# clvrai/mopa-rl

Measured on AMD Instinct MI355X. Metric: valid-state collision checks/sec, higher is better.
Workload: dtype f64; 1 GPU; SawyerPushObstacle-v0 state validity (FK + collision), 4096 envs/GPU x 256 states/env per step, states 50% uniform joint-box samples + 50% near-init N(0,0.3); envs_per_gpu=4096, states_per_env=256, parallelism=env-shard x1

## Files before the change

include/mopa_hip.h:

```cpp
#ifndef MOPA_HIP_H
#define MOPA_HIP_H
#include <stdint.h>

#ifdef __cplusplus
extern "C" {
#endif

#define MOPA_OK 0
#define MOPA_ERR_INVALID_ARG 1
#define MOPA_ERR_UNSUPPORTED 2
#define MOPA_ERR_HIP 3
#define MOPA_ERR_LIMIT 4

#define MOPA_PLAN_OK 0
#define MOPA_PLAN_NO_EXACT (-4)
#define MOPA_PLAN_INVALID_GOAL (-5)

#define MOPA_FAR 1.0e10

enum { MOPA_GEOM_PLANE = 0, MOPA_GEOM_SPHERE = 2, MOPA_GEOM_CAPSULE = 3, MOPA_GEOM_CYLINDER = 5, MOPA_GEOM_BOX = 6, MOPA_GEOM_MESH = 7 };
enum { MOPA_JNT_FREE = 0, MOPA_JNT_BALL = 1, MOPA_JNT_SLIDE = 2, MOPA_JNT_HINGE = 3 };

typedef struct MopaModel {
    int32_t nq, nbody, njnt, ngeom, npair;
// ... 71 lines not shown
                         const double *attached_dev , int64_t E, int32_t max_path, void *stream);
int mopa_scene_num_active(const MopaScene *scene);
int mopa_scene_active_idx(const MopaScene *scene, int32_t *out );
int mopa_scene_num_pairs(const MopaScene *scene);
int mopa_scene_lds_bytes(const MopaScene *scene);
int mopa_scene_valid_kernel(const MopaScene *scene, int64_t N, char *out, int32_t cap );
int mopa_scene_motion_kernel(const MopaScene *scene, int64_t N, char *out, int32_t cap );
int mopa_scene_k1_baked(const MopaScene *scene);
int mopa_scene_k1_export(const MopaSceneDesc *desc, int64_t *sizes , double *dbl, int32_t *ints, int32_t *tab, void *hdr,
                         uint64_t *fingerprint);
int mopa_scene_hdr_offset(const char *field);
int mopa_scene_k1_export_glued(const MopaSceneDesc *desc, int32_t body_a, int32_t body_b, int64_t *sizes , double *dbl, int32_t *ints,
                               int32_t *tab, void *hdr, uint64_t *fingerprint);
int mopa_k1_baked_fk_host(int index, int64_t n, const double *q_active, const double *qpos_env, double *out);
int mopa_k1_baked_resident_host(int index, int64_t n, const double *q_active, const double *qpos_env, double *out, int32_t *n_res);

int mopa_is_valid_batch(MopaScene *scene, const double *q_active_dev , const double *qpos_env_dev ,
                        int64_t N, int64_t samples_per_env, uint8_t *valid_dev , double *min_dist_dev ,
                        void *stream);
int mopa_is_valid_batch_counted(MopaScene *scene, const double *q_active_dev , const double *qpos_env_dev ,
                                int64_t N, int64_t samples_per_env, uint8_t *valid_dev , double *min_dist_dev ,
                                const int64_t *n_dev, void *stream);

int mopa_check_motion_batch(MopaScene *scene, const double *qa_dev , const double *qb_dev ,
                            const double *qpos_env_dev , int64_t N, int64_t samples_per_env,
                            uint8_t *valid_dev , void *stream);

int mopa_plan_batch(MopaScene *scene, const double *start_dev , const double *goal_dev , int64_t E,
                    const MopaPlanParams *params, double *path_dev , int32_t *path_len_dev ,
                    int32_t *status_dev , int64_t *n_checks_dev , void *stream);
// ... 395 lines not shown
```

mopa_rl_amd/_lib.py:

```python
from __future__ import annotations

import ctypes as C
import os
from typing import Optional

import numpy as np

_HERE = os.path.dirname(os.path.abspath(__file__))
LIB_PATH = os.environ.get("MOPA_HIP_LIB", os.path.join(_HERE, "csrc", "libmopa_hip.so"))

MOPA_OK = 0
MOPA_FAR = 1.0e10
PLAN_OK, PLAN_NO_EXACT, PLAN_INVALID_GOAL = 0, -4, -5

_dp = C.POINTER(C.c_double)
_ip = C.POINTER(C.c_int32)

EXPORTED_SYMBOLS = [
    "mopa_last_error", "mopa_version", "mopa_device_count", "mopa_scene_create", "mopa_scene_destroy",
    "mopa_scene_create_glued", "mopa_scene_glue", "mopa_glue_attach_batch", "mopa_glue_rows_batch", "mopa_scene_k1_export_glued",
    "mopa_scene_num_active", "mopa_scene_active_idx", "mopa_scene_num_pairs", "mopa_scene_lds_bytes", "mopa_scene_valid_kernel",
    "mopa_scene_motion_kernel",
    "mopa_scene_k1_baked", "mopa_scene_k1_export", "mopa_scene_hdr_offset", "mopa_k1_baked_fk_host", "mopa_k1_baked_resident_host",
    "mopa_is_valid_batch", "mopa_is_valid_batch_counted", "mopa_check_motion_batch", "mopa_plan_batch", "mopa_simplify_paths_batch", "mopa_simplify_paths_max_path", "mopa_shortcut_paths_batch", "mopa_shortcut_paths_max_path", "mopa_smooth_paths_batch", "mopa_smooth_paths_max_path",
    "mopa_plan_star_batch", "mopa_plan_star", "mopa_plan_star_k", "mopa_star_params_size",
    "mopa_plan_race_batch", "mopa_plan_race", "mopa_race_params_size", "mopa_pullback_batch", "mopa_is_valid_state", "mopa_plan",
    "mopa_planner_status", "mopa_debug_fk", "mopa_debug_pair_dist", "mopa_contacts_batch", "mopa_contacts_state",
    "mopa_contact_frames_batch", "mopa_contact_frames_state", "mopa_geom_frames_batch", "mopa_geom_frames_host",
    "mopa_env_create", "mopa_env_destroy", "mopa_env_obs_dim", "mopa_env_action_dim", "mopa_env_step_batch", "mopa_env_exec_batch", "mopa_env_desired_batch",
    "mopa_env_attach_dynamics", "mopa_env_attach_contacts", "mopa_env_set_contact_stats", "mopa_rollout_stage", "mopa_rollout_pool_pick", "mopa_rollout_step_size", "mopa_reuse_batch", "mopa_replay_append", "mopa_replay_sample", "mopa_ct_desc_size", "mopa_env_contact_arena", "mopa_env_dyn_dofs", "mopa_env_dyn_qvel_width", "mopa_env_dyn_forward_batch", "mopa_env_dyn_substeps_batch", "mopa_env_step_dyn_batch",
    "mopa_pusher_dyn_desc_size", "mopa_env_attach_pusher_dynamics", "mopa_env_set_pusher_stats", "mopa_env_pusher_substeps_batch",
    "mopa_env_step_pusher_batch", "mopa_env_set_contact_force",
    "mopa_ik_create", "mopa_ik_destroy", "mopa_ik_solve_batch", "mopa_ik_site_pose_batch", "mopa_ik_targets_batch",
    "mopa_ik_targets_pos_batch", "mopa_ik_displacement_pos_batch",
    "mopa_paths_unwrap_batch", "mopa_paths_unwrap_seam_batch", "mopa_paths_walk_batch", "mopa_paths_assemble_batch", "mopa_interpolate_batch",
]


# ... 230 lines not shown
    L.mopa_ik_destroy.restype = None
    L.mopa_ik_solve_batch.argtypes = [vp, C.c_int64, vp, vp, vp, C.c_double, C.c_int32, C.c_double, C.c_double, C.c_double, C.c_double,
                                      vp, vp, vp, vp]
    L.mopa_ik_site_pose_batch.argtypes = [vp, C.c_int64, vp, vp, vp, vp]
    L.mopa_ik_targets_batch.argtypes = [vp, C.c_int64, vp, vp, vp, C.c_int64, C.c_double, C.POINTER(C.c_double), C.POINTER(C.c_double), vp, vp, vp]
    L.mopa_ik_targets_pos_batch.argtypes = [vp, C.c_int64, vp, vp, C.c_int64, C.c_int32, C.c_double, C.POINTER(C.c_double), C.POINTER(C.c_double), vp, vp]
    L.mopa_ik_displacement_pos_batch.argtypes = [vp, C.c_int64, vp, vp, C.c_int64, C.c_int32, C.c_double, C.POINTER(C.c_double), C.POINTER(C.c_double),
                                                 C.c_int32, C.c_double, C.c_double, C.c_double, C.c_double, vp, vp, vp, vp, vp, vp, vp]
    L.mopa_scene_valid_kernel.argtypes = [vp, C.c_int64, C.c_char_p, C.c_int32]
    L.mopa_scene_motion_kernel.argtypes = [vp, C.c_int64, C.c_char_p, C.c_int32]
    L.mopa_scene_k1_baked.argtypes = [vp]
    L.mopa_scene_k1_export.argtypes = [vp, vp, vp, vp, vp, vp, vp]
    L.mopa_scene_hdr_offset.argtypes = [C.c_char_p]
    L.mopa_k1_baked_fk_host.argtypes = [C.c_int, C.c_int64, vp, vp, vp]
    L.mopa_k1_baked_resident_host.argtypes = [C.c_int, C.c_int64, vp, vp, vp, vp]
    i32, i64, f64 = C.c_int32, C.c_int64, C.c_double
    L.mopa_paths_unwrap_batch.argtypes = [C.c_int, i64, i32, i32, vp, i32, vp, vp, vp, f64, i32, vp, vp, vp, vp, vp, vp, vp, vp]
    L.mopa_paths_unwrap_seam_batch.argtypes = [C.c_int, i64, i32, i32, vp, i32, vp, vp, vp, f64, i32, vp, vp, vp, vp, vp, vp, vp, C.c_uint64, vp]
    L.mopa_paths_walk_batch.argtypes = [C.c_int, i64, i32, i32, vp, i32, vp, vp, f64, vp, vp, vp, vp, vp, vp, vp, vp]
    L.mopa_paths_assemble_batch.argtypes = [C.c_int, i64, i32, vp, i32, vp, vp, vp, vp, vp, vp, vp, i32, vp, vp]
    L.mopa_interpolate_batch.argtypes = [vp, i64, i32, i32, vp, vp, f64, vp, vp, vp, vp, vp]
    _lib = L
    return L


def check(rc: int) -> None:
    if rc != MOPA_OK:
        raise MopaError(f"libmopa_hip error {rc}: {lib().mopa_last_error().decode()}")


# ... 344 lines not shown
```

mopa_rl_amd/csrc/mopa_hip.hip:

```cpp
#include <hip/hip_runtime.h>

#include <algorithm>
#include <cmath>
#include <cstdio>
#include <cstdlib>
#include <cstddef>
#include <cstring>
#include <string>
#include <utility>
#include <vector>

#include <map>
#include <mutex>
#include "../../include/mopa_hip.h"
#include "mopa_device.hpp"
#include "mopa_frames.hpp"
#include "mopa_fk.hpp"
#include "mopa_host.hpp"

using namespace mopa;

static thread_local std::string g_err;
int mopa_fail(int code, const std::string &msg) {
    g_err = msg;
// ... 482 lines not shown
extern "C" int mopa_scene_k1_export_glued(const MopaSceneDesc *desc, int32_t body_a, int32_t body_b, int64_t *sizes, double *dbl, int32_t *ints,
                                          int32_t *tab, void *hdr, uint64_t *fingerprint) {
    if (body_a < 0 || body_b < 0) return fail(MOPA_ERR_INVALID_ARG, "glue: body id out of range");
    return scene_k1_export(desc, body_a, body_b, sizes, dbl, ints, tab, hdr, fingerprint);
}

extern "C" int mopa_scene_hdr_offset(const char *field) {
    if (!field) return -1;
#define MOPA_HDR_FIELD(f_) if (!std::strcmp(field, #f_)) return (int)offsetof(SceneHdr, f_);
    MOPA_HDR_FIELD(na) MOPA_HDR_FIELD(nq) MOPA_HDR_FIELD(n_pq) MOPA_HDR_FIELD(nmb) MOPA_HDR_FIELD(nmg) MOPA_HDR_FIELD(nsf)
    MOPA_HDR_FIELD(n_save) MOPA_HDR_FIELD(n_pas_b) MOPA_HDR_FIELD(n_dbl) MOPA_HDR_FIELD(n_int) MOPA_HDR_FIELD(o_mbr) MOPA_HDR_FIELD(o_mbd)
    MOPA_HDR_FIELD(o_mgd) MOPA_HDR_FIELD(o_sf_pos) MOPA_HDR_FIELD(o_sf_quat) MOPA_HDR_FIELD(o_sf_mat) MOPA_HDR_FIELD(o_act_ref)
    MOPA_HDR_FIELD(o_pq_adr) MOPA_HDR_FIELD(o_mg_geom) MOPA_HDR_FIELD(thr)
    MOPA_HDR_FIELD(o_mb_parent) MOPA_HDR_FIELD(o_chain_adr) MOPA_HDR_FIELD(o_chain_len) MOPA_HDR_FIELD(o_chain_items) MOPA_HDR_FIELD(o_g_mb)
    MOPA_HDR_FIELD(o_mb_load) MOPA_HDR_FIELD(o_mb_save) MOPA_HDR_FIELD(pfk_maxlen) MOPA_HDR_FIELD(n_gp) MOPA_HDR_FIELD(npair) MOPA_HDR_FIELD(o_pairs)
    MOPA_HDR_FIELD(o_g_rec) MOPA_HDR_FIELD(o_g_type)
#undef MOPA_HDR_FIELD
    return -1;
}

namespace {
struct K1HostSink {
    double *out;
    void operator()(int m, V3 gp, Q4 gq) {
        double *o = out + 12 * m;
        o[0] = gp.x; o[1] = gp.y; o[2] = gp.z;
        quat2mat(o + 3, gq);
    }
    void resident(int, double) {}
};
struct K1ResHostSink {
    double *out;
    void operator()(int, V3, Q4) {}
    void resident(int r, double d) { out[r] = d; }
};
template <class TR>
void k1_fk_host(int64_t n, const double *q_active, const double *qpos_env, double *out) {
    for (int64_t s = 0; s < n; s++) {
        K1HostSink sink{out + (size_t)s * 12 * TR::nmg};
        k1_fk_baked<TR>(q_active + (size_t)s * TR::na, qpos_env + (size_t)s * TR::nq, sink, std::make_integer_sequence<int, TR::nmb>{});
    }
}
template <class TR>
void k1_res_host(int64_t n, const double *q_active, const double *qpos_env, double *out) {
    for (int64_t s = 0; s < n; s++) {
        K1ResHostSink sink{out + (size_t)s * k1_n_res<TR>};
        k1_fk_baked<TR>(q_active + (size_t)s * TR::na, qpos_env + (size_t)s * TR::nq, sink, std::make_integer_sequence<int, TR::nmb>{});
    }
}
}
extern "C" int mopa_k1_baked_fk_host(int index, int64_t n, const double *q_active, const double *qpos_env, double *out) {
    if (n < 0 || (n > 0 && (!q_active || !qpos_env || !out))) return fail(MOPA_ERR_INVALID_ARG, "null argument / negative count");
#define MOPA_K1_FK_HOST(i_, T_) if (index == i_) { k1_fk_host<T_>(n, q_active, qpos_env, out); return MOPA_OK; }
    MOPA_K1_BAKED_SCENES(MOPA_K1_FK_HOST)
#undef MOPA_K1_FK_HOST
    return fail(MOPA_ERR_INVALID_ARG, "no baked scene #" + std::to_string(index));
}
extern "C" int mopa_k1_baked_resident_host(int index, int64_t n, const double *q_active, const double *qpos_env, double *out, int32_t *n_res) {
    if (n < 0 || (n > 0 && (!q_active || !qpos_env || !out))) return fail(MOPA_ERR_INVALID_ARG, "null argument / negative count");
#define MOPA_K1_RES_HOST(i_, T_) if (index == i_) { if (n_res) *n_res = k1_n_res<T_>; if (k1_n_res<T_> > 0) k1_res_host<T_>(n, q_active, qpos_env, out); return MOPA_OK; }
    MOPA_K1_BAKED_SCENES(MOPA_K1_RES_HOST)
#undef MOPA_K1_RES_HOST
    return fail(MOPA_ERR_INVALID_ARG, "no baked scene #" + std::to_string(index));
}

static int scene_create(const MopaSceneDesc *desc, int glue_a, int glue_b, MopaScene **out) {
    if (!desc || !out) return fail(MOPA_ERR_INVALID_ARG, "null argument");
    MopaScene *S = new MopaScene();
    {
        const int rc = scene_build_host(desc, S, glue_a, glue_b);
        if (rc != MOPA_OK) { delete S; return rc; }
    }
    {
        const char *eb = std::getenv("MOPA_K1_BAKED");
        const uint64_t fp = k1_fingerprint(S);
        const bool allowed = !(eb && std::string(eb) == "0") && S->k1.use_v5 && S->k1.v5_cen_lds && S->n_mesh_gp == 0 && S->glue_b < 0;
        S->k1_baked = allowed ? k1_baked_index(fp) : 0;
// ... 186 lines not shown
```

mopa_rl_amd/csrc/mopa_valid_launch.inc:

```

static int64_t k1_lane_min(const MopaScene *S) { return S->k1.v2_forced ? 64 : std::max<int64_t>(64, (int64_t)S->n_cu * 36); }
static int64_t k1_motion_expand_min(const MopaScene *S) { return S->k1.v2_forced ? 64 : std::max<int64_t>(64, (int64_t)S->n_cu * 16); }

using K1FnV1 = decltype(&k_is_valid<false, false>);
using K1FnV2 = decltype(&k_is_valid_v2<false, false>);
using K1FnV5 = decltype(&k_is_valid_v5<false, true, false>);
#define MOPA_K1_COUNT(i_, T_) +1
constexpr int kK1BakedScenes = 0 MOPA_K1_BAKED_SCENES(MOPA_K1_COUNT);
#undef MOPA_K1_COUNT

static K1FnV1 k1_kernel_v1(bool want_md, bool mesh) {
    static const K1FnV1 tab[2][2] = {{k_is_valid<false, false>, k_is_valid<true, false>}, {k_is_valid<false, true>, k_is_valid<true, true>}};
    return tab[mesh][want_md];
}
static K1FnV2 k1_kernel_v2(bool want_md, bool mesh) {
    static const K1FnV2 tab[2][2] = {{k_is_valid_v2<false, false>, k_is_valid_v2<true, false>}, {k_is_valid_v2<false, true>, k_is_valid_v2<true, true>}};
    return tab[mesh][want_md];
}
static K1FnV5 k1_kernel_v5(bool want_md, bool cen_lds, bool gate, int baked) {
    static const K1FnV5 generic[3][2] = {{k_is_valid_v5<false, true, false>, k_is_valid_v5<true, true, false>},
                                         {k_is_valid_v5<false, false, false>, k_is_valid_v5<true, false, false>},
                                         {k_is_valid_v5<false, false, true>, k_is_valid_v5<true, false, true>}};
    if (cen_lds && gate) return nullptr;
    if (!baked) return generic[cen_lds ? 0 : (gate ? 2 : 1)][want_md];
    if (!cen_lds) return nullptr;
#define MOPA_K1_CASE(i_, T_) if (baked == i_) return !want_md ? k_is_valid_v5<false, true, false, T_> : k_is_valid_v5<true, true, false, T_>;
    MOPA_K1_BAKED_SCENES(MOPA_K1_CASE)
#undef MOPA_K1_CASE
    return nullptr;
}

static void k1_register_lds() {
    auto reg = [](const void *k) { if (k) (void)hipFuncSetAttribute(k, hipFuncAttributeMaxDynamicSharedMemorySize, kMaxLdsBytes); };
    for (int md = 0; md < 2; md++)
        for (int mesh = 0; mesh < 2; mesh++) {
            reg((const void *)k1_kernel_v1(md, mesh));
            reg((const void *)k1_kernel_v2(md, mesh));
        }
    for (int md = 0; md < 2; md++)
        for (int cen_lds = 0; cen_lds < 2; cen_lds++)
            for (int gate = 0; gate < 2; gate++)
                for (int baked = 0; baked <= kK1BakedScenes; baked++) reg((const void *)k1_kernel_v5(md, cen_lds, gate, baked));
}

// ... 50 lines not shown
        p.wave_grid = grid_for(S, N);
        return p;
    }
    if (has_n_dev && !P.v2_forced && N >= v2_min && !knobs.no_dual_dispatch) {
        p.wave = true;
        p.wave_grid = grid_for(S, v2_min);
        p.n_small = v2_min;
    }
    const int64_t tiles = (N + 63) / 64;
    p.blocks = std::min<int64_t>((tiles + kWavesPerBlock - 1) / kWavesPerBlock, (int64_t)S->n_cu * 2);
    p.waves = (size_t)p.blocks * kWavesPerBlock;
    p.v5 = P.use_v5 != 0;
    p.cen_lds = P.v5_cen_lds;
    p.baked = S->k1_baked;
    p.ent_cap = want_md ? P.v5_ent_cap_md : S->hdr.v5_ent_cap;
    p.lane_lds = !p.v5 ? P.v2_lds_bytes : (want_md ? P.v5_lds_bytes_md : P.v5_lds_bytes);
    p.rows_cap = knobs.rows_cap_set ? knobs.rows_cap : std::min<long long>(std::max<long long>(4096, (long long)N / 2), 1ll << 22);
    p.gate = p.v5 && !p.cen_lds && S->n_mesh_gp > 0;
    p.rows = p.gate && p.rows_cap > 0;
    if (has_n_dev && S->n_mesh_gp > 0 && !p.gate) { p.refusal = "a device-side state count on a scene with mesh pairs needs the gated mesh pass"; return p; }
    p.rows_grid = (unsigned)(knobs.rows_blocks > 0 ? knobs.rows_blocks : 3 * S->n_cu);
    p.rows_lds = (int)((size_t)S->n_mesh_dbl * sizeof(double));
    p.mesh_pass = S->n_mesh_gp > 0;
    p.mesh_lds = P.v2_lds_bytes;
    const unsigned fb = knobs.fb_blocks > 0 ? (unsigned)knobs.fb_blocks : (p.rows ? (unsigned)std::max(1, S->n_cu / 4) : (unsigned)S->n_cu);
    p.mesh_grid = p.gate ? std::min<unsigned>((unsigned)p.blocks, fb) : (unsigned)p.blocks;
    p.debug_mesh = p.gate && knobs.debug_mesh;
    return p;
}

// ... 112 lines not shown
```

mopa_rl_amd/csrc/mopa_valid_v5.inc:

```

constexpr int kEntCapV5Max = 1024;
constexpr int kBatCapV5 = 128;
constexpr int kMprCapV5 = 128;
constexpr int kMprRow = 32;
constexpr float kCullEps = 2.0e-5f;

struct K1Generic {
    static constexpr bool kBaked = false;
};
#include "mopa_valid_v5_baked.inc"

constexpr int kResMax = 2;
#ifdef MOPA_V5_NO_RESIDENT
template <class TR> constexpr int k1_n_res = 0;
#else
template <class TR> constexpr int k1_n_res = TR::n_res;
#endif
template <class TR>
MOPA_HD constexpr bool k1_is_resident(int M, int K) {
    for (int r = 0; r < k1_n_res<TR>; r++)
        if (TR::res[r][0] == M && TR::res[r][1] == K) return true;
    return false;
}

template <class TR, int M, bool WANT_MD, int K>
MOPA_D void v5_cull_baked(float cx, float cy, float cz, const float *cen_lane, unsigned &surv_lo, unsigned &surv_hi,
                          unsigned long long &deep_mask, unsigned long long &any_kept) {
    if constexpr (!k1_is_resident<TR>(M, K)) {
    constexpr int e = TR::padr[M] + K;
    constexpr float c0 = __builtin_bit_cast(float, TR::tab[8 * e + 0]), c1 = __builtin_bit_cast(float, TR::tab[8 * e + 1]);
    constexpr float c2 = __builtin_bit_cast(float, TR::tab[8 * e + 2]), c3 = __builtin_bit_cast(float, TR::tab[8 * e + 3]);
    constexpr float c4 = __builtin_bit_cast(float, TR::tab[8 * e + 4]), c5 = __builtin_bit_cast(float, TR::tab[8 * e + 5]);
    constexpr float c6 = __builtin_bit_cast(float, TR::tab[8 * e + 6]);
    bool keep;
    if constexpr (K < TR::nmov[M]) {
        const float *pc = cen_lane + ((TR::tab[8 * e + 7] >> 14) & 0xff) * 3 * 64;
        const float dx = cx - pc[0], dy = cy - pc[64], dz = cz - pc[128];
        const float d2 = fmaf(dz, dz, fmaf(dy, dy, dx * dx));
        if constexpr (!WANT_MD && TR::tab[8 * e + 0] != 0u) deep_mask |= __ballot(d2 < c0);
        keep = !(d2 > c3);
    } else if constexpr (K < TR::nmov[M] + TR::nstat[M]) {
        const float dx = cx - c0, dy = cy - c1, dz = cz - c2;
        keep = !((fmaf(dz, dz, fmaf(dy, dy, dx * dx)) > c3) | (fabsf(dx) > c4) | (fabsf(dy) > c5) | (fabsf(dz) > c6));
    } else {
        const float dx = cx - c0, dy = cy - c1, dz = cz - c2;
        keep = !(fmaf(dz, c6, fmaf(dy, c5, dx * c4)) > c3);
    }
    if constexpr (K < 32) surv_lo |= keep ? (1u << K) : 0u;
    else surv_hi |= keep ? (1u << (K - 32)) : 0u;
    any_kept |= __ballot(keep) ? (1ull << K) : 0ull;
    }
}
template <class TR, int M, bool WANT_MD, int... K>
MOPA_D void v5_pass_a_baked(float cx, float cy, float cz, const float *cen_lane, unsigned &surv_lo, unsigned &surv_hi,
                            unsigned long long &deep_mask, unsigned long long &any_kept, std::integer_sequence<int, K...>) {
    (v5_cull_baked<TR, M, WANT_MD, K>(cx, cy, cz, cen_lane, surv_lo, surv_hi, deep_mask, any_kept), ...);
}
template <class TR, bool WANT_MD, int... M>
MOPA_D void v5_pass_a_dispatch(int m, float cx, float cy, float cz, const float *cen_lane, unsigned &surv_lo, unsigned &surv_hi,
                               unsigned long long &deep_mask, unsigned long long &any_kept, std::integer_sequence<int, M...>) {
    (void)((m == M ? (v5_pass_a_baked<TR, M, WANT_MD>(cx, cy, cz, cen_lane, surv_lo, surv_hi, deep_mask, any_kept,
                                                     std::make_integer_sequence<int, TR::pnum[M]>{}), true)
                   : false) || ...);
}

MOPA_HD constexpr double k1_bits(unsigned long long b) { return __builtin_bit_cast(double, b); }
template <class TR>
struct K1FkRegs {
    V3 pos;
    Q4 quat;
    double mat[9];
// ... 28 lines not shown
        k1_res_rec<ta>(R1, a_first ? r.res_pos[R] : gp, a_first ? r.res_quat[R] : gq, TR::res_size[R]);
        k1_res_rec<tb>(R2, a_first ? gp : r.res_pos[R], a_first ? gq : r.res_quat[R], TR::res_size[R] + 3);
        sink.resident(R, geom_dist<false>(code, R1, ta, R2, tb));
    }
}
template <class TR, int M, class Sink, int... R>
MOPA_HD void k1_fk_residents(K1FkRegs<TR> &r, const V3 &gp, const Q4 &gq, Sink &sink, std::integer_sequence<int, R...>) {
    (k1_fk_resident<TR, M, R>(r, gp, gq, sink), ...);
}
template <class TR, int M, class Sink>
MOPA_HD void k1_fk_geom(K1FkRegs<TR> &r, Sink &sink) {
    constexpr const unsigned long long *gd = TR::fk_gd[M];
    const V3 gp = add3(r.pos, mat_vec(r.mat, V3{k1_bits(gd[0]), k1_bits(gd[1]), k1_bits(gd[2])}));
    const Q4 gq = quat_mul(r.quat, Q4{k1_bits(gd[3]), k1_bits(gd[4]), k1_bits(gd[5]), k1_bits(gd[6])});
    sink(M, gp, gq);
    k1_fk_residents<TR, M>(r, gp, gq, sink, std::make_integer_sequence<int, k1_n_res<TR>>{});
}
template <class TR, int B, class Sink, int... G>
MOPA_HD void k1_fk_body(K1FkRegs<TR> &r, const double *qact, const double *sn, const double *cs, const double *pv, Sink &sink,
                        std::integer_sequence<int, G...>) {
    constexpr const int *bi = TR::fk_body[B];
    constexpr int load = bi[0], sf = bi[1], save = bi[2], mgadr = bi[3], jn = bi[5], jt = bi[6], src = bi[8];
    constexpr bool jp0 = bi[7] != 0;
    constexpr const unsigned long long *bd = TR::fk_bd[B];
    static_assert(jn <= 1 && sizeof...(G) == bi[4], "baked walk: one joint per body at most");
    if constexpr (jn == 1 && jt == J_FREE) {
        fk_free_step(pv + (src - TR::na), r.pos, r.quat);
    } else {
        V3 ppos;
        Q4 pquat;
// ... 43 lines not shown
    r.pos = V3{0.0, 0.0, 0.0};
    r.quat = Q4{1.0, 0.0, 0.0, 0.0};
    (k1_fk_body<TR, B>(r, qact, sn, cs, pv, sink, std::make_integer_sequence<int, TR::fk_body[B][4]>{}), ...);
}
struct V5FkSink {
    double *slab;
    float *cen;
    MOPA_D void operator()(int m, V3 gp, Q4 gq) {
        double *sp = slab + (size_t)m * kSlabStride;
        pose7_st<64>(sp, gp, gq);
        float *cp = cen + (size_t)m * 3 * 64;
        cp[0] = (float)gp.x; cp[64] = (float)gp.y; cp[128] = (float)gp.z;
    }
    double res_d[kResMax];
    MOPA_D void resident(int r, double d) { res_d[r] = d; }
};

struct V5Lds {
    float *cen;
    unsigned *ent;
    unsigned *bat;
    unsigned *bat2;
    unsigned long long *bad;
    unsigned long long *md;
    bool tp;
};
MOPA_HD int v5_lds_per_wave(int nmg, int ent_cap, bool want_md) { return ((nmg * 3 * 64 * 4) + ent_cap * 4 + 2 * kBatCapV5 * 4 + (want_md ? 64 * 8 : 0) + 8 + 15) & ~15; }

MOPA_D void v5_load_rec2(double (&R1)[15], double (&R2)[15], const SceneHdr &h, const double *D, const double *slab_tile,
                         int gA, int movA, int slotA, int gB, int movB, int slotB, int slA, int slB) {
// ... 168 lines not shown
        if (nd < n_small) N = 0;
    }
    extern __shared__ __attribute__((aligned(16))) unsigned char smem[];
    double *s_dbl = reinterpret_cast<double *>(smem);
    int *s_int = reinterpret_cast<int *>(s_dbl + h.n_dbl);
    int *s_tab = s_int + ((h.n_int + 3) & ~3);
    constexpr int kTail = GATE ? 3 : 1;
    for (int i = threadIdx.x; i < 8 * h.n_gp + kTail * h.nmg; i += blockDim.x) s_tab[i] = g_tab[i];
    stage_scene(h, g_dbl, g_int, s_dbl, s_int);
    LdsView v;
    v.dbl = s_dbl; v.ints = s_int; v.grec = nullptr; v.qbuf = nullptr; v.sc = nullptr; v.wl = nullptr;
    const int lane = threadIdx.x & 63, wave = threadIdx.x >> 6;
    V5Lds q;
    {
        const int n_cen = CEN_LDS ? h.nmg : 0;
        unsigned char *base = reinterpret_cast<unsigned char *>(s_tab + ((8 * h.n_gp + kTail * h.nmg + 3) & ~3)) + wave * v5_lds_per_wave(n_cen, h.v5_ent_cap, WANT_MD);
        q.cen = reinterpret_cast<float *>(base);
        q.ent = reinterpret_cast<unsigned *>(q.cen + n_cen * 3 * 64);
        q.bat = q.ent + h.v5_ent_cap;
        q.bat2 = q.bat + kBatCapV5;
        q.md = reinterpret_cast<unsigned long long *>(q.bat2 + kBatCapV5);
        q.bad = WANT_MD ? q.md + 64 : q.md;
        q.tp = false;
    }
    const double *__restrict__ GD = g_dbl;
    const int32_t *__restrict__ GI = g_int;
    const int nslab = h.nmg + h.n_save;
    double *slab = slab_all + ((size_t)blockIdx.x * kWavesPerBlock + wave) * (size_t)nslab * kSlabStride + lane;
    const double *slab_tile = slab - lane;
    double *mpr_ring = mpr_all + ((size_t)blockIdx.x * kWavesPerBlock + wave) * (size_t)kMprCapV5 * kMprRow;
    float *gcen = CEN_LDS ? nullptr : cen_all + ((size_t)blockIdx.x * kWavesPerBlock + wave) * (size_t)h.nmg * 3 * 64 + lane;
    int mpr_head = 0, mpr_count = 0;
    const long long n_tiles = (N + 63) >> 6;
// ... 6 lines not shown
        long long s = tile * 64 + lane;
        const bool act = s < N;
        if (!act) s = N - 1;
        const double *qa_row = q_active + s * h.na;
        const double *env_row = qpos_env + (env_idx ? (long long)env_idx[s] : s / samples_per_env) * h.nq;
        if (lane == 0) *q.bad = 0ull;
        if (WANT_MD) q.md[lane] = f64_sortable(0.0);

        double res_d[kResMax] = {};
#ifdef MOPA_V5_FK_REPS
        for (int fk_rep = 0; fk_rep < MOPA_V5_FK_REPS; fk_rep++)
#endif
        if constexpr (TR::kBaked) {
            double *fk_slab = slab;
            asm volatile("" : "+v"(fk_slab));
            V5FkSink sink{fk_slab, q.cen + lane, {}};
            k1_fk_baked<TR>(qa_row, env_row, sink, std::make_integer_sequence<int, TR::nmb>{});
#pragma unroll
            for (int r = 0; r < kResMax; r++) res_d[r] = sink.res_d[r];
#ifdef MOPA_V5_FK_REPS
            asm volatile("" ::: "memory");
#endif
        } else {
            double *ps = reinterpret_cast<double *>(q.ent);
            bool tile_poses = false;
            if (!GATE && h.n_pas_b > 0) {
                const unsigned long long er = (unsigned long long)env_row;
                const unsigned long long e0 = ((unsigned long long)(unsigned)__builtin_amdgcn_readfirstlane((int)(er >> 32)) << 32) | (unsigned)__builtin_amdgcn_readfirstlane((int)(unsigned)er);
                tile_poses = __all(er == e0);
            }
            q.tp = !GATE && tile_poses;
// ... 420 lines not shown
```

mopa_rl_amd/csrc/mopa_valid_v5_baked.inc:

```

struct K1Baked_SawyerPushObstacle {
    static constexpr bool kBaked = true;
    static constexpr unsigned long long kFingerprint = 0x85dfbe79baeda04bull;
    static constexpr int nmg = 14;
    static constexpr int padr[nmg] = {0, 1, 3, 4, 5, 10, 15, 29, 47, 65, 83, 101, 119, 138};
    static constexpr int pnum[nmg] = {1, 2, 1, 1, 5, 5, 14, 18, 18, 18, 18, 18, 19, 17};
    static constexpr int nmov[nmg] = {0, 0, 0, 0, 1, 1, 3, 5, 5, 5, 5, 5, 6, 13};
    static constexpr int nstat[nmg] = {0, 1, 0, 0, 3, 3, 10, 12, 12, 12, 12, 12, 12, 3};
    static constexpr int npl[nmg] = {1, 1, 1, 1, 1, 1, 1, 1, 1, 1, 1, 1, 1, 1};
    static constexpr unsigned tab[1240] = {
        0x00000000u, 0x00000000u, 0x00000000u, 0x3d8f66a5u, 0x00000000u, 0x00000000u, 0x3f800000u, 0x40001000u,
        0x00000000u, 0x00000000u, 0x3f88f5c3u, 0x3dd74fecu, 0x3e852158u, 0x3e852158u, 0x3e999c39u, 0x00000603u,
        0x00000000u, 0x00000000u, 0x00000000u, 0x3e38572au, 0x00000000u, 0x00000000u, 0x3f800000u, 0x40001000u,
        0x00000000u, 0x00000000u, 0x00000000u, 0x3e0e4865u, 0x00000000u, 0x00000000u, 0x3f800000u, 0x40001300u,
        0x00000000u, 0x00000000u, 0x00000000u, 0x3d8f66a5u, 0x00000000u, 0x00000000u, 0x3f800000u, 0x40001000u,
        0x3d67a9acu, 0x00000000u, 0x00000000u, 0x3e2c26b4u, 0x00000000u, 0x00000000u, 0x00000000u, 0x00007505u,
        0xbea66666u, 0x00000000u, 0x3f11eb85u, 0x3eac19a5u, 0x3eae171au, 0x3edc2b95u, 0x3efd7344u, 0x00000901u,
        0xbca3d70au, 0x00000000u, 0x3f28f5c3u, 0x3eb150c3u, 0x3ed1ee24u, 0x3ed1ee24u, 0x3f0a3ec0u, 0x00000b02u,
        0x00000000u, 0x00000000u, 0x3f88f5c3u, 0x3e0f6b23u, 0x3e9ebaf1u, 0x3e9ebaf1u, 0x3eb335d2u, 0x00000b03u,
        0x00000000u, 0x00000000u, 0x00000000u, 0x3e6b8a5du, 0x00000000u, 0x00000000u, 0x3f800000u, 0x40001100u,
        0x3d5e062au, 0x00000000u, 0x00000000u, 0x3db2405bu, 0x00000000u, 0x00000000u, 0x00000000u, 0x00007505u,
        0xbea66666u, 0x00000000u, 0x3f11eb85u, 0x3e5d3203u, 0x3e666ba4u, 0x3ea14a4du, 0x3ec291fcu, 0x00000901u,
        0xbca3d70au, 0x00000000u, 0x3f28f5c3u, 0x3e65928au, 0x3e970cddu, 0x3e970cddu, 0x3ed99c39u, 0x00000b02u,
        0x00000000u, 0x00000000u, 0x3f88f5c3u, 0x3d89a388u, 0x3e47b352u, 0x3e47b352u, 0x3e70a915u, 0x00000b03u,
// ... 185 lines not shown
        {0x0000000000000000ull, 0x0000000000000000ull, 0x0000000000000000ull, 0x3ff0000000000000ull, 0x0000000000000000ull, 0x0000000000000000ull, 0x0000000000000000ull},
        {0xbf989374bc6a7efaull, 0x0000000000000000ull, 0x0000000000000000ull, 0x3fe6a2ecb934b59aull, 0x0000000000000000ull, 0x3fe69e4fd79ac743ull, 0x0000000000000000ull},
        {0x0000000000000000ull, 0x0000000000000000ull, 0x0000000000000000ull, 0x3ff0000000000000ull, 0x0000000000000000ull, 0x0000000000000000ull, 0x0000000000000000ull},
        {0x0000000000000000ull, 0xbfa47ae147ae147bull, 0x0000000000000000ull, 0x3ff0000000000000ull, 0x0000000000000000ull, 0x0000000000000000ull, 0x0000000000000000ull},
        {0x0000000000000000ull, 0x0000000000000000ull, 0x0000000000000000ull, 0x3ff0000000000000ull, 0x0000000000000000ull, 0x0000000000000000ull, 0x0000000000000000ull},
    };
    static constexpr unsigned long long fk_sf[nsf][16] = {
        {0x0000000000000000ull, 0x0000000000000000ull, 0x0000000000000000ull, 0x3ff0000000000000ull, 0x0000000000000000ull, 0x0000000000000000ull, 0x0000000000000000ull, 0x3ff0000000000000ull, 0x0000000000000000ull, 0x0000000000000000ull, 0x0000000000000000ull, 0x3ff0000000000000ull, 0x0000000000000000ull, 0x0000000000000000ull, 0x0000000000000000ull, 0x3ff0000000000000ull},
        {0x0000000000000000ull, 0x0000000000000000ull, 0x3fee666666666666ull, 0x3ff0000000000000ull, 0x0000000000000000ull, 0x0000000000000000ull, 0x0000000000000000ull, 0x3ff0000000000000ull, 0x0000000000000000ull, 0x0000000000000000ull, 0x0000000000000000ull, 0x3ff0000000000000ull, 0x0000000000000000ull, 0x0000000000000000ull, 0x0000000000000000ull, 0x3ff0000000000000ull},
    };
    static constexpr unsigned long long fk_act_ref[na] = {0x0000000000000000ull, 0x0000000000000000ull, 0x0000000000000000ull, 0x0000000000000000ull, 0x0000000000000000ull, 0x0000000000000000ull, 0x0000000000000000ull};
    static constexpr int fk_pq_adr[n_pq] = {7, 8, 27, 28, 29, 30, 31, 32, 33};
    static constexpr int n_res = 1;
    static constexpr int res[1][7] = {{4, 0, 1, 4, 5, 2, 3}};
    static constexpr unsigned long long res_size[1][6] = {{0x3fc70a3d70a3d70aull, 0x0000000000000000ull, 0x0000000000000000ull, 0x3faeb851eb851eb8ull, 0x3fc5c28f5c28f5c3ull, 0x0000000000000000ull}};
};

#define MOPA_K1_BAKED_SCENES(X) X(1, K1Baked_SawyerPushObstacle)
```

Before: 2.332 billion checks/s.

## Tighten static-pair broadphase cull with orientation-dependent per-axis reach

During FK, each axis-owning moving geom now packs a 10-bit-per-component quantized local-axis direction word into LDS. Pass A uses it to compute a per-axis half-length reach and tests static pairs against tighter baked per-axis bounds instead of fixed orientation-independent extents, so fewer pairs survive to the narrowphase. The axis words take LDS space from the entry capacity, and baking is disabled if the remaining capacity would fall below 256. A host helper is added to compare old and new keep decisions.

```diff
diff --git a/include/mopa_hip.h b/include/mopa_hip.h
--- a/include/mopa_hip.h
+++ b/include/mopa_hip.h
@@ -109,6 +109,8 @@
                                int32_t *tab, void *hdr, uint64_t *fingerprint);
 int mopa_k1_baked_fk_host(int index, int64_t n, const double *q_active, const double *qpos_env, double *out);
 int mopa_k1_baked_resident_host(int index, int64_t n, const double *q_active, const double *qpos_env, double *out, int32_t *n_res);
+int mopa_k1_baked_static_host(int index, int64_t n, const double *q_active, const double *qpos_env, uint8_t *keep_new, uint8_t *keep_old,
+                              float *axis, int32_t *n_ent);
 
 int mopa_is_valid_batch(MopaScene *scene, const double *q_active_dev , const double *qpos_env_dev ,
                         int64_t N, int64_t samples_per_env, uint8_t *valid_dev , double *min_dist_dev ,
diff --git a/mopa_rl_amd/_lib.py b/mopa_rl_amd/_lib.py
--- a/mopa_rl_amd/_lib.py
+++ b/mopa_rl_amd/_lib.py
@@ -21,7 +21,7 @@
     "mopa_scene_create_glued", "mopa_scene_glue", "mopa_glue_attach_batch", "mopa_glue_rows_batch", "mopa_scene_k1_export_glued",
     "mopa_scene_num_active", "mopa_scene_active_idx", "mopa_scene_num_pairs", "mopa_scene_lds_bytes", "mopa_scene_valid_kernel",
     "mopa_scene_motion_kernel",
-    "mopa_scene_k1_baked", "mopa_scene_k1_export", "mopa_scene_hdr_offset", "mopa_k1_baked_fk_host", "mopa_k1_baked_resident_host",
+    "mopa_scene_k1_baked", "mopa_scene_k1_export", "mopa_scene_hdr_offset", "mopa_k1_baked_fk_host", "mopa_k1_baked_resident_host", "mopa_k1_baked_static_host",
     "mopa_is_valid_batch", "mopa_is_valid_batch_counted", "mopa_check_motion_batch", "mopa_plan_batch", "mopa_simplify_paths_batch", "mopa_simplify_paths_max_path", "mopa_shortcut_paths_batch", "mopa_shortcut_paths_max_path", "mopa_smooth_paths_batch", "mopa_smooth_paths_max_path",
     "mopa_plan_star_batch", "mopa_plan_star", "mopa_plan_star_k", "mopa_star_params_size",
     "mopa_plan_race_batch", "mopa_plan_race", "mopa_race_params_size", "mopa_pullback_batch", "mopa_is_valid_state", "mopa_plan",
@@ -282,6 +282,7 @@
     L.mopa_scene_hdr_offset.argtypes = [C.c_char_p]
     L.mopa_k1_baked_fk_host.argtypes = [C.c_int, C.c_int64, vp, vp, vp]
     L.mopa_k1_baked_resident_host.argtypes = [C.c_int, C.c_int64, vp, vp, vp, vp]
+    L.mopa_k1_baked_static_host.argtypes = [C.c_int, C.c_int64, vp, vp, vp, vp, vp, vp]
     i32, i64, f64 = C.c_int32, C.c_int64, C.c_double
     L.mopa_paths_unwrap_batch.argtypes = [C.c_int, i64, i32, i32, vp, i32, vp, vp, vp, f64, i32, vp, vp, vp, vp, vp, vp, vp, vp]
     L.mopa_paths_unwrap_seam_batch.argtypes = [C.c_int, i64, i32, i32, vp, i32, vp, vp, vp, f64, i32, vp, vp, vp, vp, vp, vp, vp, C.c_uint64, vp]
diff --git a/mopa_rl_amd/csrc/mopa_hip.hip b/mopa_rl_amd/csrc/mopa_hip.hip
--- a/mopa_rl_amd/csrc/mopa_hip.hip
+++ b/mopa_rl_amd/csrc/mopa_hip.hip
@@ -520,7 +520,7 @@
     MOPA_HDR_FIELD(o_pq_adr) MOPA_HDR_FIELD(o_mg_geom) MOPA_HDR_FIELD(thr)
     MOPA_HDR_FIELD(o_mb_parent) MOPA_HDR_FIELD(o_chain_adr) MOPA_HDR_FIELD(o_chain_len) MOPA_HDR_FIELD(o_chain_items) MOPA_HDR_FIELD(o_g_mb)
     MOPA_HDR_FIELD(o_mb_load) MOPA_HDR_FIELD(o_mb_save) MOPA_HDR_FIELD(pfk_maxlen) MOPA_HDR_FIELD(n_gp) MOPA_HDR_FIELD(npair) MOPA_HDR_FIELD(o_pairs)
-    MOPA_HDR_FIELD(o_g_rec) MOPA_HDR_FIELD(o_g_type)
+    MOPA_HDR_FIELD(o_g_rec) MOPA_HDR_FIELD(o_g_type) MOPA_HDR_FIELD(o_g_aabb)
 #undef MOPA_HDR_FIELD
     return -1;
 }
@@ -534,12 +534,52 @@
         quat2mat(o + 3, gq);
     }
     void resident(int, double) {}
+    void axis(int, unsigned) {}
 };
 struct K1ResHostSink {
     double *out;
     void operator()(int, V3, Q4) {}
     void resident(int r, double d) { out[r] = d; }
+    void axis(int, unsigned) {}
 };
+struct K1PassAHostSink {
+    float *cen;
+    unsigned *axw;
+    void operator()(int m, V3 gp, Q4) { cen[3 * m] = (float)gp.x; cen[3 * m + 1] = (float)gp.y; cen[3 * m + 2] = (float)gp.z; }
+    void resident(int, double) {}
+    void axis(int slot, unsigned word) { axw[slot] = word; }
+};
+template <class TR, int M, int K>
+void k1_static_host_pair(const float *c, float hx, float hy, float hz, uint8_t *keep_new, uint8_t *keep_old) {
+    if constexpr (K >= TR::nmov[M] && K < TR::nmov[M] + TR::nstat[M]) {
+        keep_new[TR::padr[M] + K] = k1_static_keep<TR, M, K, k1_axis_on<TR>>(c[0], c[1], c[2], hx, hy, hz) ? 1 : 0;
+        keep_old[TR::padr[M] + K] = k1_static_keep<TR, M, K, false>(c[0], c[1], c[2], 0.0f, 0.0f, 0.0f) ? 1 : 0;
+    }
+}
+template <class TR, int M, int... K>
+void k1_static_host_geom(const float *cen, const unsigned *axw, uint8_t *keep_new, uint8_t *keep_old, float *axis, std::integer_sequence<int, K...>) {
+    float hx = 0.0f, hy = 0.0f, hz = 0.0f;
+    if constexpr (k1_axis_owner<TR>(M)) {
+        k1_axis_unpack(axw[TR::ax_slot[M]], axis[3 * M], axis[3 * M + 1], axis[3 * M + 2]);
+        k1_axis_reach<TR, M>(axw[TR::ax_slot[M]], hx, hy, hz);
+    }
+    (k1_static_host_pair<TR, M, K>(cen + 3 * M, hx, hy, hz, keep_new, keep_old), ...);
+}
+template <class TR, int... M>
+void k1_static_host(int64_t n, const double *q_active, const double *qpos_env, uint8_t *keep_new, uint8_t *keep_old, float *axis, std::integer_sequence<int, M...>) {
+    constexpr int n_ent = (int)(sizeof(TR::tab) / (8 * sizeof(unsigned)));
+    for (int64_t s = 0; s < n; s++) {
+        float cen[3 * TR::nmg];
+        unsigned axw[k1_axis_words<TR> / 64 + 1] = {};
+        K1PassAHostSink sink{cen, axw};
+        k1_fk_baked<TR>(q_active + (size_t)s * TR::na, qpos_env + (size_t)s * TR::nq, sink, std::make_integer_sequence<int, TR::nmb>{});
+        uint8_t *kn = keep_new + (size_t)s * n_ent, *ko = keep_old + (size_t)s * n_ent;
+        float *a = axis + (size_t)s * 3 * TR::nmg;
+        std::memset(kn, 2, n_ent); std::memset(ko, 2, n_ent);
+        for (int i = 0; i < 3 * TR::nmg; i++) a[i] = -1.0f;
+        (k1_static_host_geom<TR, M>(cen, axw, kn, ko, a, std::make_integer_sequence<int, TR::pnum[M]>{}), ...);
+    }
+}
 template <class TR>
 void k1_fk_host(int64_t n, const double *q_active, const double *qpos_env, double *out) {
     for (int64_t s = 0; s < n; s++) {
@@ -567,6 +607,16 @@
 #define MOPA_K1_RES_HOST(i_, T_) if (index == i_) { if (n_res) *n_res = k1_n_res<T_>; if (k1_n_res<T_> > 0) k1_res_host<T_>(n, q_active, qpos_env, out); return MOPA_OK; }
     MOPA_K1_BAKED_SCENES(MOPA_K1_RES_HOST)
 #undef MOPA_K1_RES_HOST
+    return fail(MOPA_ERR_INVALID_ARG, "no baked scene #" + std::to_string(index));
+}
+
+extern "C" int mopa_k1_baked_static_host(int index, int64_t n, const double *q_active, const double *qpos_env, uint8_t *keep_new, uint8_t *keep_old,
+                                         float *axis, int32_t *n_ent) {
+    if (n < 0 || (n > 0 && (!q_active || !qpos_env || !keep_new || !keep_old || !axis))) return fail(MOPA_ERR_INVALID_ARG, "null argument / negative count");
+#define MOPA_K1_STATIC_HOST(i_, T_) if (index == i_) { if (n_ent) *n_ent = (int32_t)(sizeof(T_::tab) / (8 * sizeof(unsigned))); \
+        k1_static_host<T_>(n, q_active, qpos_env, keep_new, keep_old, axis, std::make_integer_sequence<int, T_::nmg>{}); return MOPA_OK; }
+    MOPA_K1_BAKED_SCENES(MOPA_K1_STATIC_HOST)
+#undef MOPA_K1_STATIC_HOST
     return fail(MOPA_ERR_INVALID_ARG, "no baked scene #" + std::to_string(index));
 }
 
diff --git a/mopa_rl_amd/csrc/mopa_valid_launch.inc b/mopa_rl_amd/csrc/mopa_valid_launch.inc
--- a/mopa_rl_amd/csrc/mopa_valid_launch.inc
+++ b/mopa_rl_amd/csrc/mopa_valid_launch.inc
@@ -28,6 +28,13 @@
     MOPA_K1_BAKED_SCENES(MOPA_K1_CASE)
 #undef MOPA_K1_CASE
     return nullptr;
+}
+
+static int k1_baked_axis_words(int baked) {
+#define MOPA_K1_AXW(i_, T_) if (baked == i_) return k1_axis_words<T_>;
+    MOPA_K1_BAKED_SCENES(MOPA_K1_AXW)
+#undef MOPA_K1_AXW
+    return 0;
 }
 
 static void k1_register_lds() {
@@ -108,6 +115,11 @@
     p.cen_lds = P.v5_cen_lds;
     p.baked = S->k1_baked;
     p.ent_cap = want_md ? P.v5_ent_cap_md : S->hdr.v5_ent_cap;
+    if (p.baked) {
+        const int ax = k1_baked_axis_words(p.baked);
+        if (p.ent_cap - ax >= 256) p.ent_cap -= ax;
+        else if (ax > 0) p.baked = 0;
+    }
     p.lane_lds = !p.v5 ? P.v2_lds_bytes : (want_md ? P.v5_lds_bytes_md : P.v5_lds_bytes);
     p.rows_cap = knobs.rows_cap_set ? knobs.rows_cap : std::min<long long>(std::max<long long>(4096, (long long)N / 2), 1ll << 22);
     p.gate = p.v5 && !p.cen_lds && S->n_mesh_gp > 0;
diff --git a/mopa_rl_amd/csrc/mopa_valid_v5.inc b/mopa_rl_amd/csrc/mopa_valid_v5.inc
--- a/mopa_rl_amd/csrc/mopa_valid_v5.inc
+++ b/mopa_rl_amd/csrc/mopa_valid_v5.inc
@@ -7,6 +7,7 @@
 
 struct K1Generic {
     static constexpr bool kBaked = false;
+    static constexpr int n_ax = 0;
 };
 #include "mopa_valid_v5_baked.inc"
 
@@ -23,8 +24,62 @@
     return false;
 }
 
+constexpr float kAxisBias = 0.02f;
+constexpr float kAxisStep = __builtin_bit_cast(float, 0x3a802009u);
+constexpr float kAxisSlack = 1.0e-3f;
+#ifdef MOPA_V5_NO_AXIS_CULL
+template <class TR> constexpr bool k1_axis_on = false;
+#else
+template <class TR> constexpr bool k1_axis_on = TR::n_ax > 0;
+#endif
+template <class TR>
+MOPA_HD constexpr bool k1_axis_owner(int M) {
+    if constexpr (k1_axis_on<TR>) return TR::ax_slot[M] >= 0;
+    else return false;
+}
+template <class TR>
+constexpr int k1_axis_words_of() {
+    if constexpr (k1_axis_on<TR>) return TR::n_ax * 64;
+    else return 0;
+}
+template <class TR> constexpr int k1_axis_words = k1_axis_words_of<TR>();
+MOPA_HD unsigned k1_axis_q10(float a) {
+    const float t = ceilf(fmaf(fabsf(a), 1023.0f, kAxisBias));
+    return t < 1023.0f ? (unsigned)t : 1023u;
+}
+MOPA_HD unsigned k1_axis_word(const Q4 &q) {
+    const float w = (float)q.w, x = (float)q.x, y = (float)q.y, z = (float)q.z;
+    const float ax = 2.0f * (x * z + w * y), ay = 2.0f * (y * z - w * x), az = ((w * w - x * x) - y * y) + z * z;
+    return k1_axis_q10(ax) | (k1_axis_q10(ay) << 10) | (k1_axis_q10(az) << 20);
+}
+MOPA_HD void k1_axis_unpack(unsigned word, float &ax, float &ay, float &az) {
+    ax = (float)(word & 1023u) * kAxisStep; ay = (float)((word >> 10) & 1023u) * kAxisStep; az = (float)(word >> 20) * kAxisStep;
+}
+template <class TR, int M>
+MOPA_HD void k1_axis_reach(unsigned word, float &hx, float &hy, float &hz) {
+    constexpr float amax = __builtin_bit_cast(float, TR::ax_max[M]), hl = __builtin_bit_cast(float, TR::ax_hl[M]);
+    k1_axis_unpack(word, hx, hy, hz);
+    hx = hl * fminf(hx, amax); hy = hl * fminf(hy, amax); hz = hl * fminf(hz, amax);
+}
+template <class TR, int M, int K, bool AXIS>
+MOPA_HD bool k1_static_keep(float cx, float cy, float cz, float hx, float hy, float hz) {
+    constexpr int e = TR::padr[M] + K;
+    constexpr float c0 = __builtin_bit_cast(float, TR::tab[8 * e + 0]), c1 = __builtin_bit_cast(float, TR::tab[8 * e + 1]);
+    constexpr float c2 = __builtin_bit_cast(float, TR::tab[8 * e + 2]), c3 = __builtin_bit_cast(float, TR::tab[8 * e + 3]);
+    const float dx = cx - c0, dy = cy - c1, dz = cz - c2;
+    if constexpr (AXIS && k1_axis_owner<TR>(M)) {
+        constexpr float e4 = __builtin_bit_cast(float, TR::ax_tab[3 * e + 0]), e5 = __builtin_bit_cast(float, TR::ax_tab[3 * e + 1]);
+        constexpr float e6 = __builtin_bit_cast(float, TR::ax_tab[3 * e + 2]);
+        return !((fmaf(dz, dz, fmaf(dy, dy, dx * dx)) > c3) | (fabsf(dx) > e4 + hx) | (fabsf(dy) > e5 + hy) | (fabsf(dz) > e6 + hz));
+    } else {
+        constexpr float c4 = __builtin_bit_cast(float, TR::tab[8 * e + 4]), c5 = __builtin_bit_cast(float, TR::tab[8 * e + 5]);
+        constexpr float c6 = __builtin_bit_cast(float, TR::tab[8 * e + 6]);
+        return !((fmaf(dz, dz, fmaf(dy, dy, dx * dx)) > c3) | (fabsf(dx) > c4) | (fabsf(dy) > c5) | (fabsf(dz) > c6));
+    }
+}
+
 template <class TR, int M, bool WANT_MD, int K>
-MOPA_D void v5_cull_baked(float cx, float cy, float cz, const float *cen_lane, unsigned &surv_lo, unsigned &surv_hi,
+MOPA_D void v5_cull_baked(float cx, float cy, float cz, const float *cen_lane, float hx, float hy, float hz, unsigned &surv_lo, unsigned &surv_hi,
                           unsigned long long &deep_mask, unsigned long long &any_kept) {
     if constexpr (!k1_is_resident<TR>(M, K)) {
     constexpr int e = TR::padr[M] + K;
@@ -40,8 +95,7 @@
         if constexpr (!WANT_MD && TR::tab[8 * e + 0] != 0u) deep_mask |= __ballot(d2 < c0);
         keep = !(d2 > c3);
     } else if constexpr (K < TR::nmov[M] + TR::nstat[M]) {
-        const float dx = cx - c0, dy = cy - c1, dz = cz - c2;
-        keep = !((fmaf(dz, dz, fmaf(dy, dy, dx * dx)) > c3) | (fabsf(dx) > c4) | (fabsf(dy) > c5) | (fabsf(dz) > c6));
+        keep = k1_static_keep<TR, M, K, k1_axis_on<TR>>(cx, cy, cz, hx, hy, hz);
     } else {
         const float dx = cx - c0, dy = cy - c1, dz = cz - c2;
         keep = !(fmaf(dz, c6, fmaf(dy, c5, dx * c4)) > c3);
@@ -54,7 +108,10 @@
 template <class TR, int M, bool WANT_MD, int... K>
 MOPA_D void v5_pass_a_baked(float cx, float cy, float cz, const float *cen_lane, unsigned &surv_lo, unsigned &surv_hi,
                             unsigned long long &deep_mask, unsigned long long &any_kept, std::integer_sequence<int, K...>) {
-    (v5_cull_baked<TR, M, WANT_MD, K>(cx, cy, cz, cen_lane, surv_lo, surv_hi, deep_mask, any_kept), ...);
+    float hx = 0.0f, hy = 0.0f, hz = 0.0f;
+    if constexpr (k1_axis_owner<TR>(M))
+        k1_axis_reach<TR, M>(reinterpret_cast<const unsigned *>(cen_lane)[(3 * TR::nmg + TR::ax_slot[M]) * 64], hx, hy, hz);
+    (v5_cull_baked<TR, M, WANT_MD, K>(cx, cy, cz, cen_lane, hx, hy, hz, surv_lo, surv_hi, deep_mask, any_kept), ...);
 }
 template <class TR, bool WANT_MD, int... M>
 MOPA_D void v5_pass_a_dispatch(int m, float cx, float cy, float cz, const float *cen_lane, unsigned &surv_lo, unsigned &surv_hi,
@@ -113,6 +170,7 @@
     const V3 gp = add3(r.pos, mat_vec(r.mat, V3{k1_bits(gd[0]), k1_bits(gd[1]), k1_bits(gd[2])}));
     const Q4 gq = quat_mul(r.quat, Q4{k1_bits(gd[3]), k1_bits(gd[4]), k1_bits(gd[5]), k1_bits(gd[6])});
     sink(M, gp, gq);
+    if constexpr (k1_axis_owner<TR>(M)) sink.axis(TR::ax_slot[M], k1_axis_word(gq));
     k1_fk_residents<TR, M>(r, gp, gq, sink, std::make_integer_sequence<int, k1_n_res<TR>>{});
 }
 template <class TR, int B, class Sink, int... G>
@@ -186,6 +244,8 @@
     }
     double res_d[kResMax];
     MOPA_D void resident(int r, double d) { res_d[r] = d; }
+    int ax_row;
+    MOPA_D void axis(int slot, unsigned word) { reinterpret_cast<unsigned *>(cen)[(ax_row + slot) * 64] = word; }
 };
 
 struct V5Lds {
@@ -384,9 +444,12 @@
     V5Lds q;
     {
         const int n_cen = CEN_LDS ? h.nmg : 0;
-        unsigned char *base = reinterpret_cast<unsigned char *>(s_tab + ((8 * h.n_gp + kTail * h.nmg + 3) & ~3)) + wave * v5_lds_per_wave(n_cen, h.v5_ent_cap, WANT_MD);
+        int ent_words = h.v5_ent_cap;
+        if constexpr (k1_axis_words<TR> > 0) ent_words += k1_axis_words<TR>;
+        unsigned char *base = reinterpret_cast<unsigned char *>(s_tab + ((8 * h.n_gp + kTail * h.nmg + 3) & ~3)) + wave * v5_lds_per_wave(n_cen, ent_words, WANT_MD);
         q.cen = reinterpret_cast<float *>(base);
         q.ent = reinterpret_cast<unsigned *>(q.cen + n_cen * 3 * 64);
+        if constexpr (k1_axis_words<TR> > 0) q.ent += k1_axis_words<TR>;
         q.bat = q.ent + h.v5_ent_cap;
         q.bat2 = q.bat + kBatCapV5;
         q.md = reinterpret_cast<unsigned long long *>(q.bat2 + kBatCapV5);
@@ -423,7 +486,7 @@
         if constexpr (TR::kBaked) {
             double *fk_slab = slab;
             asm volatile("" : "+v"(fk_slab));
-            V5FkSink sink{fk_slab, q.cen + lane, {}};
+            V5FkSink sink{fk_slab, q.cen + lane, {}, 3 * TR::nmg};
             k1_fk_baked<TR>(qa_row, env_row, sink, std::make_integer_sequence<int, TR::nmb>{});
 #pragma unroll
             for (int r = 0; r < kResMax; r++) res_d[r] = sink.res_d[r];
diff --git a/mopa_rl_amd/csrc/mopa_valid_v5_baked.inc b/mopa_rl_amd/csrc/mopa_valid_v5_baked.inc
--- a/mopa_rl_amd/csrc/mopa_valid_v5_baked.inc
+++ b/mopa_rl_amd/csrc/mopa_valid_v5_baked.inc
@@ -223,6 +223,167 @@
     static constexpr int n_res = 1;
     static constexpr int res[1][7] = {{4, 0, 1, 4, 5, 2, 3}};
     static constexpr unsigned long long res_size[1][6] = {{0x3fc70a3d70a3d70aull, 0x0000000000000000ull, 0x0000000000000000ull, 0x3faeb851eb851eb8ull, 0x3fc5c28f5c28f5c3ull, 0x0000000000000000ull}};
+    static constexpr int n_ax = 6;
+    static constexpr int ax_slot[nmg] = {-1, -1, -1, -1, 0, 1, 2, 3, 4, -1, 5, -1, -1, -1};
+    static constexpr unsigned ax_hl[nmg] = {0x00000000u, 0x00000000u, 0x00000000u, 0x00000000u, 0x3e2e147bu, 0x3d75c28fu, 0x3e19999au, 0x3d4ccccdu, 0x3ccccccdu, 0x00000000u, 0x3c75c28fu, 0x00000000u, 0x00000000u, 0x00000000u};
+    static constexpr unsigned ax_max[nmg] = {0x00000000u, 0x00000000u, 0x00000000u, 0x00000000u, 0x3f7fffffu, 0x3f7fffffu, 0x3f7ffffdu, 0x3f7ffffcu, 0x3e5dced9u, 0x00000000u, 0x3e522f11u, 0x00000000u, 0x00000000u, 0x00000000u};
+    static constexpr unsigned ax_tab[465] = {
+        0x00000000u, 0x00000000u, 0x00000000u,
+        0x00000000u, 0x00000000u, 0x00000000u,
+        0x00000000u, 0x00000000u, 0x00000000u,
+        0x00000000u, 0x00000000u, 0x00000000u,
+        0x00000000u, 0x00000000u, 0x00000000u,
+        0x00000000u, 0x00000000u, 0x00000000u,
+        0x3e2e19b9u, 0x3e852158u, 0x3ea66906u,
+        0x3e75c7ceu, 0x3e75c7ceu, 0x3ebd7343u,
+        0x3e0f6167u, 0x3e0f6167u, 0x3e38572au,
+        0x00000000u, 0x00000000u, 0x00000000u,
+        0x00000000u, 0x00000000u, 0x00000000u,
+        0x3e28fb01u, 0x3e8291fbu, 0x3ea3d9aau,
+        0x3e70a916u, 0x3e70a916u, 0x3ebae3e7u,
+        0x3e0a42afu, 0x3e0a42afu, 0x3e333871u,
+        0x00000000u, 0x00000000u, 0x00000000u,
+        0x00000000u, 0x00000000u, 0x00000000u,
+        0x00000000u, 0x00000000u, 0x00000000u,
+        0x00000000u, 0x00000000u, 0x00000000u,
+        0x3e1ebd90u, 0x3e7ae686u, 0x3e9ebaf2u,
+        0x3ee3d9aau, 0x3ee3d9aau, 0x3d852935u,
+        0x3e7ae686u, 0x3d615ca8u, 0x3e8291fcu,
+        0x3e7ae686u, 0x3d615ca8u, 0x3e8291fcu,
+        0x3e7ae686u, 0x3e666ba5u, 0x3d615ca8u,
+        0x3e7ae686u, 0x3e666ba5u, 0x3d615ca8u,
+        0x3e666ba5u, 0x3e666ba5u, 0x3eb5c52fu,
+        0x3e00053eu, 0x3e00053eu, 0x3e28fb01u,
+        0x3d852935u, 0x3d852935u, 0x3ee3d9aau,
+        0x3d852935u, 0x3d852935u, 0x3ee3d9aau,
+        0x00000000u, 0x00000000u, 0x00000000u,
+        0x00000000u, 0x00000000u, 0x00000000u,
+        0x00000000u, 0x00000000u, 0x00000000u,
+        0x00000000u, 0x00000000u, 0x00000000u,
+        0x00000000u, 0x00000000u, 0x00000000u,
+        0x00000000u, 0x00000000u, 0x00000000u,
+        0x3e1ebd90u, 0x3e7ae686u, 0x3e9ebaf2u,
+        0x3ee3d9aau, 0x3ee3d9aau, 0x3d852935u,
+        0x3e7ae686u, 0x3d615ca8u, 0x3e8291fcu,
+        0x3e7ae686u, 0x3d615ca8u, 0x3e8291fcu,
+        0x3e7ae686u, 0x3e666ba5u, 0x3d615ca8u,
+        0x3e7ae686u, 0x3e666ba5u, 0x3d615ca8u,
+        0x3e666ba5u, 0x3e666ba5u, 0x3eb5c52fu,
+        0x3e00053eu, 0x3e00053eu, 0x3e28fb01u,
+        0x3d852935u, 0x3d852935u, 0x3ee3d9aau,
+        0x3d852935u, 0x3d852935u, 0x3ee3d9aau,
+        0x3d852935u, 0x3d852935u, 0x3ee3d9aau,
+        0x3d852935u, 0x3d852935u, 0x3ee3d9aau,
+        0x00000000u, 0x00000000u, 0x00000000u,
+        0x00000000u, 0x00000000u, 0x00000000u,
+        0x00000000u, 0x00000000u, 0x00000000u,
+        0x00000000u, 0x00000000u, 0x00000000u,
+        0x00000000u, 0x00000000u, 0x00000000u,
+        0x00000000u, 0x00000000u, 0x00000000u,
+        0x3e28fb01u, 0x3e8291fbu, 0x3ea3d9aau,
+        0x3e70a916u, 0x3e70a916u, 0x3ebae3e7u,
+        0x3e0a42afu, 0x3e0a42afu, 0x3e333871u,
+        0x3ee8f862u, 0x3ee8f862u, 0x3d99a416u,
+        0x3d99a416u, 0x3d99a416u, 0x3ee8f862u,
+        0x3d99a416u, 0x3d99a416u, 0x3ee8f862u,
+        0x3d99a416u, 0x3d99a416u, 0x3ee8f862u,
+        0x3d99a416u, 0x3d99a416u, 0x3ee8f862u,
+        0x3e8291fbu, 0x3d852935u, 0x3e87b0b4u,
+        0x3e8291fbu, 0x3d852935u, 0x3e87b0b4u,
+        0x3e8291fbu, 0x3e70a916u, 0x3d852935u,
+        0x3e8291fbu, 0x3e70a916u, 0x3d852935u,
+        0x00000000u, 0x00000000u, 0x00000000u,
+        0x00000000u, 0x00000000u, 0x00000000u,
+        0x00000000u, 0x00000000u, 0x00000000u,
+        0x00000000u, 0x00000000u, 0x00000000u,
+        0x00000000u, 0x00000000u, 0x00000000u,
+        0x00000000u, 0x00000000u, 0x00000000u,
+        0x00000000u, 0x00000000u, 0x00000000u,
+        0x00000000u, 0x00000000u, 0x00000000u,
+        0x00000000u, 0x00000000u, 0x00000000u,
+        0x00000000u, 0x00000000u, 0x00000000u,
+        0x00000000u, 0x00000000u, 0x00000000u,
+        0x00000000u, 0x00000000u, 0x00000000u,
+        0x00000000u, 0x00000000u, 0x00000000u,
+        0x00000000u, 0x00000000u, 0x00000000u,
+        0x00000000u, 0x00000000u, 0x00000000u,
+        0x00000000u, 0x00000000u, 0x00000000u,
+        0x00000000u, 0x00000000u, 0x00000000u,
+        0x00000000u, 0x00000000u, 0x00000000u,
+        0x00000000u, 0x00000000u, 0x00000000u,
+        0x00000000u, 0x00000000u, 0x00000000u,
+        0x00000000u, 0x00000000u, 0x00000000u,
+        0x00000000u, 0x00000000u, 0x00000000u,
+        0x00000000u, 0x00000000u, 0x00000000u,
+        0x00000000u, 0x00000000u, 0x00000000u,
+        0x3e148020u, 0x3e70a916u, 0x3e999c39u,
+        0x3e5c2e34u, 0x3e5c2e34u, 0x3eb0a676u,
+        0x3deb8f9bu, 0x3deb8f9bu, 0x3e1ebd90u,
+        0x3edebaf1u, 0x3edebaf1u, 0x3d615ca8u,
+        0x3d615ca8u, 0x3d615ca8u, 0x3edebaf1u,
+        0x3d615ca8u, 0x3d615ca8u, 0x3edebaf1u,
+        0x3d615ca8u, 0x3d615ca8u, 0x3edebaf1u,
+        0x3d615ca8u, 0x3d615ca8u, 0x3edebaf1u,
+        0x3e70a916u, 0x3d3866e5u, 0x3e7ae686u,
+        0x3e70a916u, 0x3d3866e5u, 0x3e7ae686u,
+        0x3e70a916u, 0x3e5c2e34u, 0x3d3866e5u,
+        0x3e70a916u, 0x3e5c2e34u, 0x3d3866e5u,
+        0x00000000u, 0x00000000u, 0x00000000u,
+        0x00000000u, 0x00000000u, 0x00000000u,
+        0x00000000u, 0x00000000u, 0x00000000u,
+        0x00000000u, 0x00000000u, 0x00000000u,
+        0x00000000u, 0x00000000u, 0x00000000u,
+        0x00000000u, 0x00000000u, 0x00000000u,
+        0x00000000u, 0x00000000u, 0x00000000u,
+        0x00000000u, 0x00000000u, 0x00000000u,
+        0x00000000u, 0x00000000u, 0x00000000u,
+        0x00000000u, 0x00000000u, 0x00000000u,
+        0x00000000u, 0x00000000u, 0x00000000u,
+        0x00000000u, 0x00000000u, 0x00000000u,
+        0x00000000u, 0x00000000u, 0x00000000u,
+        0x00000000u, 0x00000000u, 0x00000000u,
+        0x00000000u, 0x00000000u, 0x00000000u,
+        0x00000000u, 0x00000000u, 0x00000000u,
+        0x00000000u, 0x00000000u, 0x00000000u,
+        0x00000000u, 0x00000000u, 0x00000000u,
+        0x00000000u, 0x00000000u, 0x00000000u,
+        0x00000000u, 0x00000000u, 0x00000000u,
+        0x00000000u, 0x00000000u, 0x00000000u,
+        0x00000000u, 0x00000000u, 0x00000000u,
+        0x00000000u, 0x00000000u, 0x00000000u,
+        0x00000000u, 0x00000000u, 0x00000000u,
+        0x00000000u, 0x00000000u, 0x00000000u,
+        0x00000000u, 0x00000000u, 0x00000000u,
+        0x00000000u, 0x00000000u, 0x00000000u,
+        0x00000000u, 0x00000000u, 0x00000000u,
+        0x00000000u, 0x00000000u, 0x00000000u,
+        0x00000000u, 0x00000000u, 0x00000000u,
+        0x00000000u, 0x00000000u, 0x00000000u,
+        0x00000000u, 0x00000000u, 0x00000000u,
+        0x00000000u, 0x00000000u, 0x00000000u,
+        0x00000000u, 0x00000000u, 0x00000000u,
+        0x00000000u, 0x00000000u, 0x00000000u,
+        0x00000000u, 0x00000000u, 0x00000000u,
+        0x00000000u, 0x00000000u, 0x00000000u,
+        0x00000000u, 0x00000000u, 0x00000000u,
+        0x00000000u, 0x00000000u, 0x00000000u,
+        0x00000000u, 0x00000000u, 0x00000000u,
+        0x00000000u, 0x00000000u, 0x00000000u,
+        0x00000000u, 0x00000000u, 0x00000000u,
+        0x00000000u, 0x00000000u, 0x00000000u,
+        0x00000000u, 0x00000000u, 0x00000000u,
+        0x00000000u, 0x00000000u, 0x00000000u,
+        0x00000000u, 0x00000000u, 0x00000000u,
+        0x00000000u, 0x00000000u, 0x00000000u,
+        0x00000000u, 0x00000000u, 0x00000000u,
+        0x00000000u, 0x00000000u, 0x00000000u,
+        0x00000000u, 0x00000000u, 0x00000000u,
+        0x00000000u, 0x00000000u, 0x00000000u,
+        0x00000000u, 0x00000000u, 0x00000000u,
+        0x00000000u, 0x00000000u, 0x00000000u,
+        0x00000000u, 0x00000000u, 0x00000000u,
+        0x00000000u, 0x00000000u, 0x00000000u,
+    };
 };
 
 #define MOPA_K1_BAKED_SCENES(X) X(1, K1Baked_SawyerPushObstacle)
```

After: 2.389 billion checks/s, median of 6. 1.02x the previous value.
